# regeirk/pycwt

Hardware: NVIDIA H100
Metric: cwt_scale_points_per_sec (higher is better)
Workload: dtype f64

## Files before the change

### pycwt_b200/csrc/cplx.cuh

```cuda
#pragma once
#include <cuda_runtime.h>

#ifndef HD
#ifdef CWTB_HOST_EMU
#define HD inline
#else
#define HD __host__ __device__ __forceinline__
#endif
#endif

namespace cwtb {

template <typename T> struct Vec2;
template <> struct Vec2<double> { using type = double2; };
template <> struct Vec2<float> { using type = float2; };
template <typename T> using cx = typename Vec2<T>::type;

template <typename T> HD cx<T> mk(T a, T b) {
  cx<T> r; r.x = a; r.y = b; return r;
}
template <typename V> HD V cadd(V a, V b) { a.x += b.x; a.y += b.y; return a; }
template <typename V> HD V csub(V a, V b) { a.x -= b.x; a.y -= b.y; return a; }
template <typename V> HD V cmul(V a, V b) {
  V r;
  r.x = a.x * b.x - a.y * b.y;
  r.y = a.x * b.y + a.y * b.x;
  return r;
}
template <typename V> HD V cconj(V a) { a.y = -a.y; return a; }
template <int SIGN, typename V> HD V mul_si(V a) {
  V r;
  if (SIGN > 0) { r.x = -a.y; r.y = a.x; } else { r.x = a.y; r.y = -a.x; }
  return r;
}
template <typename V, typename T> HD V cscale(V a, T s) { a.x *= s; a.y *= s; return a; }

HD void sincospi_hd(double x, double *s, double *c) {
#if defined(__CUDA_ARCH__) && !defined(CWTB_HOST_EMU)
  sincospi(x, s, c);
#else
  ::sincos(3.14159265358979323846 * x, s, c);
#endif
}

HD void sincos_hd(double x, double *s, double *c) {
#if defined(__CUDA_ARCH__) && !defined(CWTB_HOST_EMU)
  sincos(x, s, c);
#else
  ::sincos(x, s, c);
#endif
}

HD double norm2_rn(double re, double im) {
#if defined(__CUDA_ARCH__) && !defined(CWTB_HOST_EMU)
  return __dadd_rn(__dmul_rn(re, re), __dmul_rn(im, im));
#else
  return re * re + im * im;
#endif
}

template <int SIGN, typename V> HD void dft2(V &a, V &b) {
  V t = csub(a, b);
  a = cadd(a, b);
  b = t;
}

template <int SIGN, typename V>
HD void dft4(V &x0, V &x1, V &x2, V &x3) {
  V t0 = cadd(x0, x2), t1 = csub(x0, x2);
  V t2 = cadd(x1, x3), t3 = mul_si<SIGN>(csub(x1, x3));
  x0 = cadd(t0, t2);
  x2 = csub(t0, t2);
  x1 = cadd(t1, t3);
  x3 = csub(t1, t3);
}

template <int SIGN, typename T, typename V> HD V mul_w8_1(V a) {
  const T h = (T)0.70710678118654752440;
  V r;
  if (SIGN > 0) { r.x = (a.x - a.y) * h; r.y = (a.x + a.y) * h; }
  else          { r.x = (a.x + a.y) * h; r.y = (a.y - a.x) * h; }
  return r;
}
template <int SIGN, typename T, typename V> HD V mul_w8_3(V a) {
  const T h = (T)0.70710678118654752440;
  V r;
  if (SIGN > 0) { r.x = (-a.x - a.y) * h; r.y = (a.x - a.y) * h; }
  else          { r.x = (a.y - a.x) * h; r.y = (-a.x - a.y) * h; }
  return r;
}
// ... 76 lines not shown
```

### pycwt_b200/csrc/engine.cu

```cuda
#include <algorithm>
#include <array>
#include <cmath>
#include <cstdint>
#include <cstdio>
#include <cstdlib>
#include <cstring>
#include <map>
#include <mutex>
#include <set>
#include <string>
#include <type_traits>
#include <vector>

#include <cuda_runtime.h>
#include <dlfcn.h>
#include <initializer_list>

#include "../../include/cwt_b200.h"
#include "kernels.cuh"

using namespace cwtb;

template <class B, class = void> struct BodyNT { static constexpr int value = NT; };
template <class B> struct BodyNT<B, std::void_t<decltype(B::NTB)>> { static constexpr int value = B::NTB; };
// ... 1435 lines not shown
                 &c->C, &c->A12, &c->F, &c->aux, &c->rowd, &c->win, &c->mask, &c->hist, &c->noise, &c->wide, &c->blueA, &c->blueX, &c->blueY, &c->pspec, &c->prot, &c->coh.buf, &c->cross.buf, &c->coh3.buf, &c->coh.counts, &c->coh3.counts})
    if (b->p) rt_free(b->p);
  for (auto &kv : c->ntabs) { rt_free(kv.second.hi); rt_free(kv.second.lo); }
  for (auto &kv : c->blue) { rt_free(kv.second.wm); rt_free(kv.second.bf[0]); rt_free(kv.second.bf[1]); }
  if (c->tw64) rt_free(c->tw64);
  if (c->tw32) rt_free(c->tw32);
  for (void *p : c->pinned) rt_host_free(p);
  for (void *p : c->devallocs) rt_free(p);
  rt_event_destroy(c->e0);
  rt_event_destroy(c->e1);
  rt_stream_destroy(c->stream);
  for (auto &st : c->copy_streams) rt_stream_destroy(st);
  rt_stream_destroy(c->aux_stream);
  rt_stream_destroy(c->prio_stream);
  rt_stream_destroy(c->prio_short);
  rt_event_destroy(c->ev_angle);
  rt_event_destroy(c->ev_coarse);
  rt_event_destroy(c->ev_coarse_short);
  for (auto &ev : c->ev_h2d) rt_event_destroy(ev);
  for (auto &ev : c->ev_used) rt_event_destroy(ev);
  for (void *p : c->stage_host) if (p) rt_host_free(p);
  for (auto &st : c->chain_streams) rt_stream_destroy(st);
  for (auto &ev : c->ev_joinc) rt_event_destroy(ev);
  rt_event_destroy(c->ev_fork);
  rt_event_destroy(c->ev_join);
  delete c;
}

const char *cwtb_last_error(cwtb_ctx *c) { return c ? c->err.c_str() : "null context"; }

int cwtb_set_band_eps(cwtb_ctx *c, double eps) {
  if (!c || !(eps >= 0) || eps >= 1e-6) return fail(c, CWTB_ERR_ARG, "band eps must be in [0, 1e-6)");
  c->band_eps = eps;
  return 0;
}

int cwtb_set_expand_eps(cwtb_ctx *c, double eps64, double eps32) {
  if (!c || !(eps64 >= 0) || !(eps32 >= 0) || eps64 > 1e-6 || eps32 > 1e-3)
    return fail(c, CWTB_ERR_ARG, "expansion tolerance must be in [0, 1e-6] (fp64) / [0, 1e-3] (fp32)");
  c->expand_eps = eps64;
  c->expand_eps32 = eps32;
  return 0;
}

int cwtb_host_alloc(cwtb_ctx *c, size_t bytes, void **out) {
  if (!c || !out) return CWTB_ERR_ARG;
  if (rt_host_alloc(out, bytes) != 0) return fail(c, CWTB_ERR_NOMEM, "pinned allocation failed");
  c->pinned.insert(*out);
  return 0;
}
int cwtb_host_free(cwtb_ctx *c, void *p) {
  if (!c || !c->pinned.count(p)) return CWTB_ERR_ARG;
  c->pinned.erase(p);
  rt_host_free(p);
  return 0;
}
int cwtb_dev_alloc(cwtb_ctx *c, size_t bytes, void **out) {
  if (!c || !out) return CWTB_ERR_ARG;
  if (rt_malloc(out, bytes) != 0) return fail(c, CWTB_ERR_NOMEM, "device allocation failed");
  c->devallocs.insert(*out);
  return 0;
}
int cwtb_dev_free(cwtb_ctx *c, void *p) {
  if (!c || !c->devallocs.count(p)) return CWTB_ERR_ARG;
  c->devallocs.erase(p);
  rt_free(p);
  return 0;
}
int cwtb_memcpy_h2d(cwtb_ctx *c, void *dst, const void *src, size_t bytes) {
  RT(rt_h2d(dst, src, bytes, c->stream));
  RT(rt_sync(c->stream));
  return 0;
}
int cwtb_memcpy_d2h(cwtb_ctx *c, void *dst, const void *src, size_t bytes) {
  RT(rt_d2h(dst, src, bytes, c->stream));
  RT(rt_sync(c->stream));
  return 0;
}
int cwtb_sync(cwtb_ctx *c) {
  RT(rt_sync(c->stream));
  return 0;
}

static const double kOsUs = 9.5;
static const double kTwoKernelUs = 23.2;

struct DevTmp {
  void *p = nullptr;
  ~DevTmp() { if (p) rt_free(p); }
};

static int os_plan(cwtb_ctx *c, const Job &job, double dt, int family, double param, std::vector<OsRow> &os) {
  constexpr int L = OsBody<4>::L, GR = 4;
  auto os_cheaper = [](int M) { return M <= L / 2 && kOsUs * L / (double)(L - M + 1) < kTwoKernelUs; };
  os.assign(job.S, OsRow());
  const unsigned N = job.N;
  if (!c->os_on || job.precision != CWTB_F64 || job.exact || family == CWTB_TABLE ||
      !(c->band_eps > 0) || !(c->expand_eps > 0) || N < 2u * L)
    return 0;
  const long long half = (long long)N / 2;
  std::vector<int> cand;
  std::vector<double> cs;
  for (const ScaleDesc &d : job.descs) {
    if (d.chan != 0 || d.k_hi < d.k_lo || d.k_lo <= -half || d.k_hi >= ((long long)N - 1) / 2) continue;
    if (d.ip_log2Nc || (d.log2K <= 10 || (d.log2K <= DIRECT_MAX_LOG2 && d.log2K < job.log2N))) continue;
    cand.push_back(d.row);
    cs.push_back(d.s);
  }
  if (cand.empty()) return 0;
  const int nc = (int)cand.size();
  const size_t wcap = (size_t)job.S * job.nbatch * job.n0;
  const int chunk = (int)std::max<size_t>(1, wcap / N);
  int e = ensure(c, c->W, std::max<size_t>((size_t)chunk * N, wcap) * sizeof(double2));
  if (e) return e;
  double2 *h = (double2 *)c->W.p;
  DevTmp dimp, part;
  if (rt_malloc(&dimp.p, (size_t)N * sizeof(double))) return fail(c, CWTB_ERR_NOMEM, "device allocation failed");
  {
    std::vector<double> delta(N, 0.0);
    delta[0] = 1.0;
    RT(rt_h2d(dimp.p, delta.data(), (size_t)N * sizeof(double), c->stream));
    RT(rt_sync(c->stream));
  }
  const int nblk = 64;
  if (rt_malloc(&part.p, (size_t)chunk * nblk * sizeof(double))) return fail(c, CWTB_ERR_NOMEM, "device allocation failed");
  std::vector<double> farmax(nc, 0.0);
  std::vector<double2> win((size_t)nc * 2 * L);
  for (int r0 = 0; r0 < nc; r0 += chunk) {
    const int nr = std::min(chunk, nc - r0);
    Job imp;
    const double xeps = c->expand_eps;
    c->expand_eps = 0;
    e = build_job(c, imp, (long long)N, dt, cs.data() + r0, nr, family, param, CWTB_F64, false, 1);
    c->expand_eps = xeps;
    if (e) return e;
    if ((e = upload_descs(c, imp))) return e;
    if ((e = run_job<double>(c, imp, (const double *)dimp.p, h, EPI_STORE))) return e;
    if (N > 2u * L) {
      AbsMaxArgs aa{h, (double *)part.p, (long long)N, (long long)L, (long long)N - L, nblk};
      if ((e = launch<AbsMaxBody>(c, nblk, nr, aa))) return e;
      std::vector<double> ph((size_t)nr * nblk);
      RT(rt_d2h(ph.data(), part.p, ph.size() * sizeof(double), c->stream));
      RT(rt_sync(c->stream));
      for (int r = 0; r < nr; ++r)
        for (int b = 0; b < nblk; ++b) farmax[r0 + r] = std::max(farmax[r0 + r], ph[(size_t)r * nblk + b]);
    }
    for (int r = 0; r < nr; ++r) {
      RT(rt_d2h(&win[(size_t)(r0 + r) * 2 * L], h + (size_t)r * N + (N - L), L * sizeof(double2), c->stream));
      RT(rt_d2h(&win[(size_t)(r0 + r) * 2 * L + L], h + (size_t)r * N, L * sizeof(double2), c->stream));
    }
    RT(rt_sync(c->stream));
  }
  struct Acc { int r, t0, t1; };
  std::vector<Acc> acc;
  std::vector<double> m(2 * L), pre(2 * L + 1);
  for (int r = 0; r < nc; ++r) {
    const double2 *w = &win[(size_t)r * 2 * L];
    double mx = farmax[r];
    for (int i = 0; i < 2 * L; ++i) mx = std::max(mx, std::max(std::fabs(w[i].x), std::fabs(w[i].y)));
    const double ulp = 2.220446049250313e-16 * mx;
    if (!(mx > 0) || farmax[r] > 128 * ulp) continue;
    const double floor_ = std::max(2 * farmax[r], 8 * ulp);
    double l1 = 0;
    pre[0] = 0;
    for (int i = 0; i < 2 * L; ++i) {
      const double a = std::hypot(w[i].x, w[i].y);
      l1 += a;
      m[i] = std::max(std::fabs(w[i].x), std::fabs(w[i].y)) > floor_ ? a : 0.0;
// ... 1846 lines not shown
```

### pycwt_b200/csrc/fft_tile.cuh

```cuda
#pragma once
#include "cplx.cuh"

namespace cwtb {

#ifndef CWTB_NT
#define CWTB_NT 128
#endif
#ifndef CWTB_NT_F32
#define CWTB_NT_F32 256
#endif
#ifndef CWTB_TILE_F64
#define CWTB_TILE_F64 4096
#endif
#ifndef CWTB_TILE_F32
#define CWTB_TILE_F32 8192
#endif
#ifndef CWTB_MINB
#define CWTB_MINB 1
#endif
#ifndef CWTB_UNROLL_B
#define CWTB_UNROLL_B 1
#endif
#define CWTB_STR_(x) #x
#define CWTB_STR(x) CWTB_STR_(x)
// ... 265 lines not shown
  }
  HD void load(int, V (&x)[R]) {
    if (ONE_SHOT) {
      V e = nroot_t<T>(nt, (unsigned)base * pp);
      const V se = nroot_t<T>(nt, (unsigned)stride * pp);
      const V ne = nroot_t<T>(nt, (unsigned)(-K) * pp);
#pragma unroll
      for (int i = 0; i < R; ++i) {
        const int r = base + i * stride;
        x[i] = cmul(ldg(&B[r]), (r >= rsplit) ? cmul(e, ne) : e);
        e = cmul(e, se);
      }
      return;
    }
#pragma unroll
    for (int i = 0; i < R; ++i) { x[i] = a[ONE_SHOT ? 0 : i]; a[ONE_SHOT ? 0 : i] = cmul(a[ONE_SHOT ? 0 : i], d[ONE_SHOT ? 0 : i]); }
  }
};

template <typename T, int K, int L, int R, int SIGN, class Loader, bool ROWS = false>
HD void pass_mid(cx<T> *sm, const cx<T> *__restrict__ tw, Loader &ld, int tid) {
  using V = cx<T>;
  using LY = Lay<T, K, ROWS>;
  constexpr int NT = TileCfg<T>::NT;
  constexpr int Ln = L / R, I = K / R, P = LY::P;
  constexpr int LANES = (I >= NT) ? NT : I;
  constexpr int GROUPS = NT / LANES;
  const int tp0 = tid % LANES, bg = tid / LANES;
  for (int tp = tp0; tp < I; tp += LANES) {
    const int g = tp / Ln, j = tp % Ln;
    V twv[R];
#pragma unroll
    static_assert(tw_radix(L) == R, "pass twiddle table was built for another radix");
    for (int c = 1; c < R; ++c) {
      V w = ldg(&tw[tw_offset(L) + (c - 1) * Ln + j]);
      if (SIGN < 0) w.y = -w.y;
      twv[c] = w;
    }
    ld.begin(g * L + j, Ln, bg, GROUPS);
    CWTB_PRAGMA_UNROLL_B
    for (int b = bg; b < P; b += GROUPS) {
      V x[R];
      ld.load(b, x);
      dftR<R, SIGN, T>(x);
#pragma unroll
      for (int c = 1; c < R; ++c) x[c] = cmul(x[c], twv[c]);
#pragma unroll
      for (int c = 0; c < R; ++c) sm[LY::phys(b, g * L + c * Ln + j)] = x[c];
    }
  }
}

template <typename T, int K, int SIGN, class Storer, bool ROWS = false, bool GMAJOR = false>
HD void pass_last(const cx<T> *sm, Storer &st, int tid) {
  using V = cx<T>;
  using LY = Lay<T, K, ROWS>;
  constexpr int NT = TileCfg<T>::NT;
  constexpr int R = Plan<K>::RL, G = K / R, P = LY::P;
  for (int idx = tid; idx < G * P; idx += NT) {
    const int b = GMAJOR ? idx / G : idx % P, g = GMAJOR ? idx % G : idx / P;
    V x[R];
#pragma unroll
    for (int i = 0; i < R; ++i) x[i] = sm[LY::phys(b, g * R + i)];
    dftR<R, SIGN, T>(x);
    st.store(b, Plan<K>::qlow(g), G, x);
  }
}

template <typename T, int K> struct TilePhases {
  static constexpr int NP = Plan<K>::NP;
};

template <typename T, int K, int SIGN, class Loader, bool ROWS = false>
HD void tile_first(cx<T> *sm, const cx<T> *tw, Loader &ld, int tid) {
  pass_mid<T, K, K, Plan<K>::R1, SIGN, Loader, ROWS>(sm, tw, ld, tid);
}
template <typename T, int K, int SIGN, bool ROWS = false>
HD void tile_second(cx<T> *sm, const cx<T> *tw, int tid) {
  SmemLoader<T, K, ROWS> ld;
  ld.sm = sm;
  pass_mid<T, K, K / Plan<K>::R1, Plan<K>::R2, SIGN, SmemLoader<T, K, ROWS>, ROWS>(sm, tw, ld, tid);
}

}
```

### pycwt_b200/csrc/kernels.cuh

```cuda
#pragma once
#include <math.h>
#include "fft_tile.cuh"

namespace cwtb {

struct ScaleDesc {
  double s;
  double amp;
  int row;
  int k_lo, k_hi;
  int log2K;
  int rsplit;
  int trow;
  int chan;
  int pad_;
  long long boff;
  int ip_log2Nc;
  int ip_kc;
  int ip_w;
  int os_grp;
  long long ip_coff;
  long long ip_woff;
  double ip_beta;
  double ip_dc;
// ... 252 lines not shown
            for (int r1 = 0; r1 < K1; ++r1)
              acc = cadd(acc, cmul(bv[r1], wt[(b * 2 + (neg[r1] ? 1 : 0)) * K1 + r1]));
            sm[LY::phys(b, r2)] = cmul(acc, t);
            t = cmul(t, dr);
          }
          e = cmul(e, se);
          dr = cmul(dr, sdr);
        }
      } else
      for (int it0 = 0; it0 < NIT; it0 += IB) {
        V bv[IB][K1], t[IB], dd[IB];
#pragma unroll
        for (int q = 0; q < IB; ++q) {
          const int r2 = tid + NT * (it0 + q);
#pragma unroll
          for (int r1 = 0; r1 < K1; ++r1) bv[q][r1] = ldg(&B[r1 * K + r2]);
          t[q] = e;
          dd[q] = dr;
          e = cmul(e, se);
          dr = cmul(dr, sdr);
        }
#pragma unroll
        for (int b = 0; b < P; ++b) {
          V acc[IB];
#pragma unroll
          for (int q = 0; q < IB; ++q) acc[q] = mk<T>(0, 0);
#pragma unroll
          for (int r1 = 0; r1 < K1; ++r1) {
            if (r1 != r1s) {
              const V w = wt[(b * 2 + (r1 > r1s ? 1 : 0)) * K1 + r1];
#pragma unroll
              for (int q = 0; q < IB; ++q) acc[q] = cadd(acc[q], cmul(bv[q][r1], w));
            } else {
              const V wp = wt[(b * 2 + 0) * K1 + r1], wn = wt[(b * 2 + 1) * K1 + r1];
#pragma unroll
              for (int q = 0; q < IB; ++q) {
                const bool neg = (tid + NT * (it0 + q)) >= r2s;
                acc[q] = cadd(acc[q], cmul(bv[q][r1], neg ? wn : wp));
              }
            }
          }
#pragma unroll
          for (int q = 0; q < IB; ++q) {
            sm[LY::phys(b, tid + NT * (it0 + q))] = cmul(acc[q], t[q]);
            t[q] = cmul(t[q], dd[q]);
          }
        }
      }
    } else if constexpr (PH == 2) {
      SmemLoader<T, K> ld;
      ld.sm = sm;
      tile_first<T, K, +1>(sm, a.tw, ld, tid);
    } else if constexpr (PH == 3 && NP == 3) {
      tile_second<T, K, +1>(sm, a.tw, tid);
    } else {
      OutStorer<T> st;
      st.row = a.W + (size_t)d.row * a.n0;
      st.nout = a.n0;
      st.u0 = u0;
      st.U = U;
      st.epi.mode = a.epi;
      pass_last<T, K, +1>(sm, st, tid);
    }
  }
};

template <typename T> struct PassBArgs {
  const cx<T> *Z;
  cx<T> *out;
  const cx<T> *tw;
  const ScaleDesc *descs;
  const double *grow;
  long long pitch, nout;
  double post;
  unsigned N;
  int first, row0;
  int epi;
  int pf_dist;
  int ny;
  int by0;
  int ileave;
};

template <typename T, int SIGN, int K2 = K2C> struct PassBBody {
  static constexpr int NTB = TileCfg<T>::NT;
  static constexpr int NT = NTB;
  using V = cx<T>;
  using Args = PassBArgs<T>;
  static constexpr int K = K2;
  using LY = Lay<T, K, true>;
  static constexpr int NP = Plan<K>::NP;
  static constexpr int NPHASE = NP + 1;
  static constexpr size_t SMEM = LY::TILE_BYTES + 16;
  static constexpr bool ROWS_ALIGNED = (LY::PITCH * sizeof(V)) % 16 == 0;
  template <int PH> HD static void phase(const Args &a, int bx, int by, int tid, void *smraw) {
    static_assert(ROWS_ALIGNED, "PassB: tile rows must start on 16-byte boundaries");
    const int ey = by;
    by = a.ny - 1 - ey;
    V *sm = (V *)smraw;
    const int U = (int)(a.N / K);
    const int u0 = bx * LY::P;
    TileBarrier tb;
    tb.bar = (unsigned long long *)((char *)smraw + LY::TILE_BYTES);
    if constexpr (PH == 0) {
      const int nvalid = (U - u0) < LY::P ? (U - u0) : LY::P;
      const V *src = a.Z + (size_t)by * a.N + (size_t)u0 * K;
      if (tid == 0) {
        tb.init_and_expect((unsigned)(nvalid * K * sizeof(V)));
        for (int b = 0; b < nvalid; ++b)
          tb.copy(sm + LY::phys(b, 0), src + (size_t)b * K, (unsigned)(K * sizeof(V)));
      }
      if (tid == 0 && a.pf_dist > 0) {
        long long t = (long long)bx + a.pf_dist;
        int pe = ey;
        const int tiles = (U + LY::P - 1) / LY::P;
        while (t >= tiles && pe + 1 < a.ny) { t -= tiles; ++pe; }
        const int py = a.ny - 1 - pe;
        if (t < tiles && t * LY::P + LY::P <= U)
          TileBarrier::prefetch_l2(a.Z + (size_t)py * a.N + (size_t)t * LY::P * K,
                                   (unsigned)(LY::P * K * sizeof(V)));
      }
      for (int b = nvalid; b < LY::P; ++b)
        for (int i = tid; i < K; i += NT) sm[LY::phys(b, i)] = mk<T>(0, 0);
    } else if constexpr (PH == 1) {
      tb.wait(0);
      SmemLoader<T, K, true> ld;
      ld.sm = sm;
      tile_first<T, K, SIGN, SmemLoader<T, K, true>, true>(sm, a.tw, ld, tid);
    } else if constexpr (PH == 2 && NP == 3) {
      tile_second<T, K, SIGN, true>(sm, a.tw, tid);
    } else {
      const int il = a.ileave > 1 ? a.ileave : 1;
      const int outer = (a.by0 + by) / il;
      const int row = a.descs ? a.descs[a.first + outer].row : a.row0 + outer;
      OutStorer<T> st;
      st.row = a.out + (size_t)row * a.pitch;
      st.nout = a.nout;
      st.u0 = u0;
      st.U = U;
      st.ostride = il;
      st.ooff = (a.by0 + by) % il;
      st.epi.mode = a.epi;
      if (a.epi == EPI_GAUSS) {
        st.epi.g = a.grow[row];
        st.epi.invn = 1.0 / ((double)a.N * il);
        st.epi.post = a.post;
        st.epi.nfreq = (long long)a.N * il;
      }
      pass_last<T, K, SIGN, OutStorer<T>, true>(sm, st, tid);
      if (tid == 0) tb.inval();
    }
  }
};

struct OsGroup {
  int first, count;
  int t1, hop;
  long long hoff;
};
struct OsArgs {
  const ScaleDesc *descs;
  const OsGroup *groups;
  const double *sig;
  const double2 *H;
  double2 *W;
  const double2 *tw;
  long long n0;
  unsigned N;
  int epi;
};

template <int L, int R> struct OsSigLoader {
  const double *x;
  long long start, n0;
  unsigned nmask;
  int hop, base, stride;
  HD void begin(int base_, int stride_, int, int) { base = base_; stride = stride_; }
  HD void load(int b, double2 (&v)[R]) const {
    const long long s = start + (long long)b * hop + base;
#pragma unroll
    for (int i = 0; i < R; ++i) {
      const long long n = (s + (long long)i * stride) & (long long)nmask;
      v[i] = make_double2(n < n0 ? ldg(&x[n]) : 0.0, 0.0);
    }
  }
};
template <int L> struct OsHalfStorer {
  double2 *xs;
  template <int R> HD void store(int b, int ql, int qs, double2 (&x)[R]) const {
#pragma unroll
    for (int c = 0; c < R; ++c) {
      const int q = ql + c * qs;
      if (q <= L / 2) xs[b * (L / 2 + 1) + q] = x[c];
    }
  }
};
template <int L, int R> struct OsSpecLoader {
  const double2 *xs, *H;
  int base, stride;
  double2 hv[R];
  HD void begin(int base_, int stride_, int, int) {
    base = base_; stride = stride_;
#pragma unroll
    for (int i = 0; i < R; ++i) hv[i] = ldg(&H[base + i * stride]);
  }
  HD void load(int b, double2 (&v)[R]) const {
#pragma unroll
    for (int i = 0; i < R; ++i) {
      const int q = base + i * stride;
      const double2 y = q <= L / 2 ? xs[b * (L / 2 + 1) + q] : cconj(xs[b * (L / 2 + 1) + L - q]);
      v[i] = cmul(y, hv[i]);
    }
  }
};
struct OsStorer {
  double2 *row;
  long long nb0, n0;
  int t1, hop, epi;
  template <int R> HD void store(int b, int ql, int qs, double2 (&x)[R]) const {
    const long long nb = nb0 + (long long)b * hop;
#pragma unroll
    for (int c = 0; c < R; ++c) {
      const int i = ql + c * qs;
      const long long n = nb + i;
      if (i >= t1 && i < t1 + hop && n < n0) {
        if (epi == EPI_STORE) st_stream(&row[n], x[c]);
        else row[n] = cmul(row[n], cconj(x[c]));
      }
    }
  }
};

template <int G> struct OsBody {
  static constexpr int L = 1024;
  static constexpr int NTB = TileCfg<double>::NT;
  static constexpr int NT = NTB;
  using Args = OsArgs;
  using LY = Lay<double, L>;
  static constexpr int P = LY::P;
  static_assert(Plan<L>::NP == 3, "overlap-save phases assume a three-pass tile plan");
  static constexpr int NPHASE = 3 + 3 * G;
  static constexpr size_t SMEM = LY::TILE_BYTES + (size_t)P * (L / 2 + 1) * sizeof(double2);
  template <int PH> HD static void phase(const Args &a, int bx, int by, int tid, void *smraw) {
    double2 *sm = (double2 *)smraw;
    double2 *xs = (double2 *)((char *)smraw + LY::TILE_BYTES);
    const OsGroup g = a.groups[by];
    const long long n_first = (long long)bx * P * g.hop;
    if (n_first >= a.n0) return;
    if constexpr (PH == 0) {
      OsSigLoader<L, Plan<L>::R1> ld;
      ld.x = a.sig + (size_t)a.descs[g.first].chan * a.n0; ld.start = n_first - g.t1; ld.n0 = a.n0; ld.nmask = a.N - 1; ld.hop = g.hop;
      tile_first<double, L, -1>(sm, a.tw, ld, tid);
    } else if constexpr (PH == 1) {
      tile_second<double, L, -1>(sm, a.tw, tid);
    } else if constexpr (PH == 2) {
      OsHalfStorer<L> st{xs};
      pass_last<double, L, -1, OsHalfStorer<L>, false, true>(sm, st, tid);
    } else {
      constexpr int r = (PH - 3) / 3, step = (PH - 3) % 3;
      if (r >= g.count) return;
      if constexpr (step == 0) {
        OsSpecLoader<L, Plan<L>::R1> ld;
        ld.xs = xs; ld.H = a.H + g.hoff + (long long)r * L;
        tile_first<double, L, +1>(sm, a.tw, ld, tid);
      } else if constexpr (step == 1) {
        tile_second<double, L, +1>(sm, a.tw, tid);
      } else {
        OsStorer st;
        st.row = a.W + (size_t)a.descs[g.first + r].row * a.n0;
        st.nb0 = n_first - g.t1; st.n0 = a.n0; st.t1 = g.t1; st.hop = g.hop; st.epi = a.epi;
        pass_last<double, L, +1, OsStorer, false, true>(sm, st, tid);
      }
    }
  }
};

struct AbsMaxArgs { const double2 *h; double *out; long long pitch, lo, hi; int nblk; };
struct AbsMaxBody {
  using Args = AbsMaxArgs;
  static constexpr int NPHASE = 2;
  static constexpr size_t SMEM = NT * sizeof(double);
  template <int PH> HD static void phase(const Args &a, int bx, int by, int tid, void *smraw) {
    double *sm = (double *)smraw;
    if constexpr (PH == 0) {
      const long long chunk = (a.hi - a.lo + a.nblk - 1) / a.nblk;
      const long long s = a.lo + bx * chunk, e = s + chunk < a.hi ? s + chunk : a.hi;
      double m = 0;
      for (long long i = s + tid; i < e; i += NT) {
        const double2 v = a.h[(size_t)by * a.pitch + i];
        m = fmax(m, fmax(fabs(v.x), fabs(v.y)));
      }
      sm[tid] = m;
    } else if (tid == 0) {
      double m = 0;
      for (int i = 0; i < NT; ++i) m = fmax(m, sm[i]);
      a.out[(size_t)by * a.nblk + bx] = m;
    }
  }
};

enum { MODE_DENSE = 0, MODE_BAND = 1, MODE_REAL = 2, MODE_CPLX = 3, MODE_COARSE = 4 };

template <typename T> HD cx<T> coarse_value(const Fam &fam, const ScaleDesc &d, const cx<T> *spec, int r, unsigned Nx) {
  const int Nc = 1 << d.ip_log2Nc;
  const int kp = r < Nc / 2 ? r : r - Nc;
  const int k = d.ip_kc + kp;
  if (k < d.k_lo || k > d.k_hi) return mk<T>(0, 0);
  const cx<T> b = band_value<T>(fam, d, spec, (unsigned)k & (Nx - 1), k, Nx);
  const double pw = 3.14159265358979323846 * (double)d.ip_w;
  const double x = pw * ((double)kp / (double)Nc);
  const double bb = d.ip_beta * d.ip_beta;
  const double z = sqrt(fma(-x, x, bb));
  const double f = d.ip_dc * (z / sinh(z));
  return mk<T>((T)((double)b.x * f), (T)((double)b.y * f));
}

template <typename T> struct PassAArgs {
  const ScaleDesc *descs;
  const cx<T> *spec;
  const cx<T> *Bbuf;
  const void *in;
  cx<T> *Z;
  const cx<T> *tw;
  Fam fam;
  NTab nt;
  long long in_pitch, n_in;
  unsigned N;
  int first, row0;
  int pf_dist;
  unsigned K2;
  unsigned Nx;
};

template <typename T, int K1, int MODE, int SIGN> struct PassABody {
  static constexpr int NTB = TileCfg<T>::NT;
  static constexpr int NT = NTB;
  using V = cx<T>;
  using Args = PassAArgs<T>;
  using LY = Lay<T, K1>;
  static constexpr int NP = Plan<K1>::NP;
  static constexpr int P = LY::P;
  static constexpr int T2 = P < K2C ? P : K2C;
  static constexpr int NPHASE = NP == 1 ? 1 : NP + 1;
  static constexpr size_t SMEM = LY::BYTES;

  struct Src {
    const Args &a;
    ScaleDesc d;
    int by, p;
    V twist0;
    HD Src(const Args &a_, int by_, int p_) : a(a_), by(by_), p(p_) {
      if (MODE == MODE_DENSE || MODE == MODE_BAND || MODE == MODE_COARSE) d = a.descs[a.first + by];
    }
    HD V get(int pos, int r2) const {
      const unsigned r = (unsigned)pos * a.K2 + (unsigned)r2;
      if (MODE == MODE_DENSE) {
        const int k = (int)r - (r >= a.N / 2 ? (int)a.N : 0);
        if (a.fam.family != 3 && (k < d.k_lo || k > d.k_hi)) return mk<T>(0, 0);
        return band_value<T>(a.fam, d, a.spec, r, k, a.N);
      } else if (MODE == MODE_BAND) {
        V v = ldg(&a.Bbuf[d.boff + r]);
        if (p == 0 || NP > 1) return v;
        const int k1 = pos - ((int)r >= d.rsplit ? K1 : 0);
        V w = nroot_t<T>(a.nt, (unsigned)k1 * (unsigned)p * a.K2);
        return cmul(v, w);
      } else if (MODE == MODE_COARSE) {
        return coarse_value<T>(a.fam, d, a.spec, (int)r, a.Nx);
      } else if (MODE == MODE_REAL) {
        const T *row = (const T *)a.in + (size_t)(a.row0 + by) * a.in_pitch;
        return mk<T>((long long)r < a.n_in ? ldg(&row[r]) : (T)0, (T)0);
      } else {
        const V *row = (const V *)a.in + (size_t)(a.row0 + by) * a.in_pitch;
        return (long long)r < a.n_in ? ldg(&row[r]) : mk<T>(0, 0);
      }
    }
  };

  template <int PH> HD static void phase(const Args &a, int bx, int by, int tid, void *smraw) {
    V *sm = (V *)smraw;
    const int NTILE2 = (int)(a.K2 / T2);
    const int p = bx / NTILE2;
    const int r20 = (bx % NTILE2) * T2;
    const int M = (int)(a.N / ((unsigned)K1 * a.K2));
    ZStorer<T, SIGN> st;
    st.Z = a.Z + (size_t)by * a.N;
    st.nt = a.nt;
    st.p = p;
    st.M = M;
    st.r20 = r20;
    st.bmax = T2;
    st.K2 = a.K2;
    if constexpr (NP == 1) {
      Src src(a, by, p);
      for (int b = tid; b < T2; b += NT) {
        V x[K1];
#pragma unroll
        for (int i = 0; i < K1; ++i) x[i] = src.get(i, r20 + b);
        dftR<K1, SIGN, T>(x);
        st.store(b, 0, 1, x);
      }
    } else if constexpr (PH == 0) {
      Src src(a, by, p);
      if (MODE == MODE_BAND && a.pf_dist > 0 && T2 * sizeof(V) >= 256) {
        const int tiles = M * NTILE2;
        const int t = bx + a.pf_dist;
        if (t < tiles) {
          const int r20n = (t % NTILE2) * T2;
          const V *base = a.Bbuf + src.d.boff + r20n;
          for (int pos = tid; pos < K1; pos += NT)
            TileBarrier::prefetch_l2(base + (size_t)pos * a.K2, (unsigned)(T2 * sizeof(V)));
        }
      }
      if (MODE == MODE_CPLX && a.pf_dist > 0 && T2 * sizeof(V) >= 256) {
        const int t = bx + a.pf_dist;
        if (t < M * NTILE2) {
          const V *row = (const V *)a.in + (size_t)(a.row0 + by) * a.in_pitch + (t % NTILE2) * T2;
          for (int pos = tid; pos < K1; pos += NT)
            if ((long long)pos * a.K2 + (t % NTILE2) * T2 + T2 <= a.n_in)
              TileBarrier::prefetch_l2(row + (size_t)pos * a.K2, (unsigned)(T2 * sizeof(V)));
        }
      }
      if (MODE == MODE_DENSE && a.fam.family == 0 && T2 <= NT) {
        constexpr int DPOS = NT / T2;
        const ScaleDesc &d = src.d;
        const int b = tid % T2;
        const long long D = (long long)DPOS * a.K2;
        const double wd = 6.283185307179586 * ((double)D * a.fam.dw);
        const double aa = d.s * wd;
        const double q = exp(-aa * aa);
        double g = 0, rho = 0;
        long long kprev = 0;
        int since = 1 << 30;
        constexpr int UB = CWTB_PASSA_BATCH;
        const V *sp = a.spec + (size_t)d.chan * a.N + (unsigned)(r20 + b);
        for (int pos0 = tid / T2; pos0 < K1; pos0 += DPOS * UB) {
          V raw[UB];
          int kk[UB];
#pragma unroll
          for (int u = 0; u < UB; ++u) {
            const int pos = pos0 + u * DPOS;
            const unsigned r = (unsigned)pos * a.K2 + (unsigned)(r20 + b);
            const int k = (int)r - (r >= a.N / 2 ? (int)a.N : 0);
            const bool in = pos < K1 && k >= d.k_lo && k <= d.k_hi;
            kk[u] = in ? k : (int)0x7fffffff;
            raw[u] = in ? ldg(&sp[(size_t)pos * a.K2]) : mk<T>(0, 0);
          }
#pragma unroll
          for (int u = 0; u < UB; ++u) {
            const int pos = pos0 + u * DPOS;
            if (pos >= K1) break;
            V v = mk<T>(0, 0);
            if (kk[u] != (int)0x7fffffff) {
              const int k = kk[u];
              if (since >= 16 || (long long)k != kprev + D || g < 1e-290) {
                const double f = d.s * (6.283185307179586 * ((double)k * a.fam.dw));
                const double dd = f - a.fam.f0;
                g = exp(-0.5 * dd * dd);
                rho = exp(-aa * dd - 0.5 * aa * aa);
                since = 0;
              } else {
                g *= rho;
                rho *= q;
                ++since;
              }
              kprev = k;
              v = cscale(raw[u], (T)(g * d.amp));
            } else {
              since = 1 << 30;
            }
            sm[LY::phys(b, pos)] = v;
          }
        }
      } else {
        CWTB_PRAGMA_UNROLL_A
        for (int idx = tid; idx < K1 * T2; idx += NT) {
          const int b = idx % T2, pos = idx / T2;
          sm[LY::phys(b, pos)] = src.get(pos, r20 + b);
        }
      }
    } else if constexpr (PH == 1) {
      if (MODE == MODE_BAND && p != 0) {
        SmemTwistLoader<T, K1, Plan<K1>::R1> ld;
        ld.sm = sm;
        ld.nt = a.nt;
        ld.rsplit_row = a.descs[a.first + by].rsplit / (int)a.K2;
        ld.pk2 = (unsigned)p * a.K2;
        tile_first<T, K1, SIGN>(sm, a.tw, ld, tid);
      } else {
        SmemLoader<T, K1> ld;
        ld.sm = sm;
        tile_first<T, K1, SIGN>(sm, a.tw, ld, tid);
      }
    } else if constexpr (PH == 2 && NP == 3) {
      tile_second<T, K1, SIGN>(sm, a.tw, tid);
    } else {
      pass_last<T, K1, SIGN>(sm, st, tid);
    }
  }
};

struct CoarseSeg { int first, count, log2Nc, cta0; };
constexpr int CSEG_MAX = 32;
HD constexpr size_t cmax(size_t a, size_t b) { return a > b ? a : b; }
template <typename T> struct CoarseArgs {
  const ScaleDesc *descs;
  const cx<T> *spec;
  cx<T> *Z;
  cx<T> *C;
  const cx<T> *tw;
  Fam fam;
  NTab nt[11];
  unsigned Nx;
  int nseg;
  int pf_dist;
  CoarseSeg seg[CSEG_MAX];
};
template <typename T> HD const CoarseSeg &coarse_seg(const CoarseArgs<T> &a, int bx) {
  int s = 0;
  while (s + 1 < a.nseg && bx >= a.seg[s + 1].cta0) ++s;
  return a.seg[s];
}

template <typename T> struct CoarseRowsBody {
  static constexpr int NTB = TileCfg<T>::NT;
  static constexpr int NT = NTB;
  using V = cx<T>;
  using Args = CoarseArgs<T>;
  template <int K> static constexpr size_t bytes() { return Lay<T, K>::BYTES; }
  static constexpr size_t SMEM = cmax(cmax(cmax(bytes<64>(), bytes<128>()), cmax(bytes<256>(), bytes<512>())), bytes<1024>());
  static constexpr int NPHASE = 4;
  HD static int ctas(int log2Nc, int rows) {
    const int P = TileCfg<T>::TILE >> log2Nc;
    return (rows + P - 1) / P;
  }
  struct Storer {
    V *out;
    int nb;
    int K;
    template <int R> HD void store(int b, int ql, int qs, V (&x)[R]) const {
      if (b >= nb) return;
#pragma unroll
      for (int c = 0; c < R; ++c) out[(size_t)b * K + ql + c * qs] = x[c];
    }
  };
  template <int K, int PH> HD static void tile(const Args &a, const CoarseSeg &g, int bx, int tid, V *sm) {
    using LY = Lay<T, K>;
    constexpr int NP = Plan<K>::NP;
    static_assert(NP >= 2, "coarse rows: multi-pass tile plans only");
    const int row0 = (bx - g.cta0) * LY::P;
    const int nb = g.count - row0 < LY::P ? g.count - row0 : LY::P;
    if constexpr (PH == 0) {
      for (int idx = tid; idx < LY::P * K; idx += NT) {
        const int b = idx / K, pos = idx % K;
        V v = mk<T>(0, 0);
        if (b < nb) v = coarse_value<T>(a.fam, a.descs[g.first + row0 + b], a.spec, pos, a.Nx);
        sm[LY::phys(b, pos)] = v;
      }
    } else if constexpr (PH == 1) {
      SmemLoader<T, K> ld;
      ld.sm = sm;
      tile_first<T, K, +1>(sm, a.tw, ld, tid);
    } else if constexpr (PH == 2 && NP == 3) {
      tile_second<T, K, +1>(sm, a.tw, tid);
    } else if constexpr (PH == NP) {
      Storer st{a.C + a.descs[g.first].ip_coff + (size_t)row0 * K, nb, K};
      pass_last<T, K, +1>(sm, st, tid);
    }
  }
  template <int PH> HD static void phase(const Args &a, int bx, int, int tid, void *smraw) {
    const CoarseSeg &g = coarse_seg(a, bx);
    V *sm = (V *)smraw;
    switch (g.log2Nc) {
      case 6: tile<64, PH>(a, g, bx, tid, sm); break;
      case 7: tile<128, PH>(a, g, bx, tid, sm); break;
      case 8: tile<256, PH>(a, g, bx, tid, sm); break;
      case 9: tile<512, PH>(a, g, bx, tid, sm); break;
      case 10: tile<1024, PH>(a, g, bx, tid, sm); break;
    }
  }
};

template <typename T> struct CoarseABody {
  static constexpr int NTB = TileCfg<T>::NT;
  static constexpr int NT = NTB;
  using V = cx<T>;
  using Args = CoarseArgs<T>;
  template <int K1> using A = PassABody<T, K1, MODE_COARSE, +1>;
  static constexpr size_t SMEM = cmax(cmax(cmax(cmax(A<2>::SMEM, A<4>::SMEM), cmax(A<8>::SMEM, A<16>::SMEM)),
                                           cmax(cmax(A<32>::SMEM, A<64>::SMEM), cmax(A<128>::SMEM, A<256>::SMEM))),
                                      cmax(A<512>::SMEM, A<1024>::SMEM));
  static constexpr int NPHASE = 4;
  template <int K1> HD static int per_row() { return K2C / A<K1>::T2; }
  HD static int ctas(int log2Nc, int rows) {
    switch (log2Nc - 10) {
      case 1: return rows * per_row<2>();
      case 2: return rows * per_row<4>();
      case 3: return rows * per_row<8>();
      case 4: return rows * per_row<16>();
      case 5: return rows * per_row<32>();
      case 6: return rows * per_row<64>();
      case 7: return rows * per_row<128>();
      case 8: return rows * per_row<256>();
      case 9: return rows * per_row<512>();
      case 10: return rows * per_row<1024>();
    }
    return 0;
  }
  template <int K1, int PH> HD static void tile(const Args &a, const CoarseSeg &g, int bx, int tid, void *sm) {
    if constexpr (PH < A<K1>::NPHASE) {
      const int local = bx - g.cta0, per = per_row<K1>();
      PassAArgs<T> pa{};
      pa.descs = a.descs; pa.spec = a.spec; pa.tw = a.tw; pa.fam = a.fam; pa.nt = a.nt[g.log2Nc - 10];
      pa.Z = a.Z + a.descs[g.first].ip_coff;
      pa.N = 1u << g.log2Nc; pa.Nx = a.Nx; pa.first = g.first; pa.K2 = K2C;
      A<K1>::template phase<PH>(pa, local % per, local / per, tid, sm);
    }
  }
  template <int PH> HD static void phase(const Args &a, int bx, int, int tid, void *sm) {
    const CoarseSeg &g = coarse_seg(a, bx);
    switch (g.log2Nc - 10) {
      case 1: tile<2, PH>(a, g, bx, tid, sm); break;
      case 2: tile<4, PH>(a, g, bx, tid, sm); break;
      case 3: tile<8, PH>(a, g, bx, tid, sm); break;
      case 4: tile<16, PH>(a, g, bx, tid, sm); break;
      case 5: tile<32, PH>(a, g, bx, tid, sm); break;
      case 6: tile<64, PH>(a, g, bx, tid, sm); break;
      case 7: tile<128, PH>(a, g, bx, tid, sm); break;
      case 8: tile<256, PH>(a, g, bx, tid, sm); break;
      case 9: tile<512, PH>(a, g, bx, tid, sm); break;
      case 10: tile<1024, PH>(a, g, bx, tid, sm); break;
    }
  }
};

template <typename T> struct CoarseBBody {
  using B = PassBBody<T, +1>;
  static constexpr int NTB = B::NTB;
  static constexpr int NT = NTB;
  using Args = CoarseArgs<T>;
  static constexpr size_t SMEM = B::SMEM;
  static constexpr int NPHASE = B::NPHASE;
  HD static int per_row(int log2Nc) {
    constexpr int P = B::LY::P;
    return ((1 << (log2Nc - 10)) + P - 1) / P;
  }
  HD static int ctas(int log2Nc, int rows) { return rows * per_row(log2Nc); }
  template <int PH> HD static void phase(const Args &a, int bx, int, int tid, void *sm) {
    const CoarseSeg &g = coarse_seg(a, bx);
    const int local = bx - g.cta0, per = per_row(g.log2Nc);
    const long long off = a.descs[g.first].ip_coff;
    const unsigned Nc = 1u << g.log2Nc;
    PassBArgs<T> pb{};
    pb.Z = a.Z + off; pb.out = a.C + off; pb.tw = a.tw;
    pb.pitch = Nc; pb.nout = Nc; pb.N = Nc; pb.post = 1.0;
    pb.epi = EPI_STORE; pb.pf_dist = a.pf_dist; pb.ny = g.count; pb.ileave = 1;
    B::template phase<PH>(pb, local % per, local / per, tid, sm);
  }
};

template <typename T> struct ExpandArgs {
  const ScaleDesc *descs;
  const cx<T> *C;
  const double *wt;
  cx<T> *W;
  NTab nt;
  long long n0;
  unsigned N;
  int first;
  int epi;
  int log2N;
};

template <typename T, int TAPS, int EPI = EPI_STORE> struct ExpandBody {
  static constexpr int NTB = TileCfg<T>::NT;
  static constexpr int NT = NTB;
  static constexpr int MINB = sizeof(T) == 8 ? 4 : 2;
  using V = cx<T>;
  using Args = ExpandArgs<T>;
  static constexpr int L = 32;
  static constexpr int MINR = 4;
  static constexpr int MAXRUN = NT / MINR;
  static constexpr int STAGE = MAXRUN * L + TAPS;
  HD static int skew(int i) { return i + (i >> 5); }
  static constexpr int NPHASE = 2;
  static constexpr size_t SMEM = (size_t)(STAGE + STAGE / 32 + 2) * sizeof(V);
  template <int PH> HD static void phase(const Args &a, int bx, int by, int tid, void *smraw) {
    V *sm = (V *)smraw;
    const ScaleDesc &d = a.descs[a.first + by];
    const int log2R = a.log2N - d.ip_log2Nc;
    const int R = 1 << log2R;
    const int Nc = 1 << d.ip_log2Nc;
    const int RB = R < NT ? R : NT;
    const int NRUN = NT / RB;
    const int MT = NRUN * L;
    const int mtiles = (Nc + MT - 1) / MT;
    const int mt = bx % mtiles, rb = bx / mtiles;
    if (rb * RB >= R) return;
    const int m0 = mt * MT;
    if constexpr (PH == 0) {
      const V *c = a.C + d.ip_coff;
      for (int i = tid; i < MT + TAPS; i += NT) {
        const int m = (m0 - (TAPS / 2 - 1) + i) & (Nc - 1);
        sm[skew(i)] = ldg(&c[m]);
      }
    } else {
      const int rl = tid & (RB - 1), j = tid / RB;
      const int rho = rb * RB + rl;
      const int ms = m0 + j * L;
      const long long nfirst = ((long long)ms << log2R) + rho;
      long long keep = (a.n0 - nfirst + R - 1) >> log2R;
      if (keep > Nc - ms) keep = Nc - ms;
      const int smax = keep < 0 ? 0 : (keep > L ? L : (int)keep);
      if (smax == 0) return;
      T hw[TAPS];
      const double *wt = a.wt + d.ip_woff + rho;
#pragma unroll
      for (int t = 0; t < TAPS; ++t) hw[t] = (T)ldg(&wt[(size_t)t * R]);
      const V *run = sm + 33 * j;
      V win[TAPS];
// ... 1423 lines not shown
```

Baseline: 110.2 billion.

## Use register-resident 32x32 FFT core for 1024-point fp64 tiles

Adds a register-resident 1024-point FFT core (radix-32 in registers, one shared-memory transpose with padded rows and fused twiddles) and uses it in the dense pass A, pass B, and the overlap-save kernel in place of the three-pass shared-memory tile plan. This cuts phases and block barriers per tile and shrinks shared-memory traffic. In exchange each thread holds 32 complex doubles, which raises register pressure, and some helpers are marked noinline to keep code size down. The overlap-save cost constants are retuned so the planner picks overlap-save more often.

```diff
diff --git a/profiles/micro/x32_ab.py b/profiles/micro/x32_ab.py
--- /dev/null
+++ b/profiles/micro/x32_ab.py
@@ -0,0 +1,81 @@
+import os
+import subprocess
+import sys
+
+import numpy as np
+
+ROOT = os.path.dirname(os.path.dirname(os.path.dirname(os.path.abspath(__file__))))
+sys.path.insert(0, ROOT)
+import workloads as wl
+from pycwt_b200 import _engine
+from bench import pin_to_gpu_numa_node
+
+CORE = (("OsBody", "OsBody<4>"), ("dense first", "PassABody<double, 1024, 0, 1>"),
+        ("second", "PassBBody<double, 1, 1024"))
+
+
+def main():
+    args = sys.argv[1:]
+    parent = args[0]
+    new = args[1] if len(args) > 1 and not args[1].isdigit() else os.path.join(ROOT, "pycwt_b200", "libcwtb200.so")
+    rounds = int(args[-1]) if args[-1].isdigit() else 8
+    pin_to_gpu_numa_node(0)
+    print(subprocess.run(["nvidia-smi", "--query-gpu=name,power.limit,clocks.max.sm", "--format=csv"],
+                         capture_output=True, text=True).stdout.strip())
+    c = wl.C2
+    x = wl.config2_signal()
+    sj = wl.config2_scales()
+    arms = {"parent": _engine.Engine(0, lib_path=parent), "new": _engine.Engine(0, lib_path=new)}
+    dev = {}
+    for name, eng in arms.items():
+        d = eng.dev_alloc(x.nbytes)
+        eng.h2d(d, x)
+        eng.cwt_dev(d, 0, c["n"], c["dt"], sj, _engine.MORLET, c["f0"], _engine.F64)
+        eng.bench_last(10)
+        dev[name] = d
+        plan = eng.last_plan(len(sj))
+        os_rows = [j for j, p in enumerate(plan) if p == -2]
+        print("%-6s plan: %d overlap-save rows (%s), %d expansion, %d exact" % (
+            name, len(os_rows), "%d..%d" % (os_rows[0], os_rows[-1]) if os_rows else "-",
+            sum(p < -2 for p in plan), sum(p >= 0 for p in plan)))
+    times = {k: [] for k in arms}
+    for _ in range(rounds):
+        for name, eng in arms.items():
+            times[name].append(eng.bench_last(20))
+    for name, t in times.items():
+        print("%-6s config 2 step %.4f ms (min %.4f, max %.4f) over %d runs of 20 steps" % (
+            name, float(np.median(t)), min(t), max(t), len(t)))
+    print("median difference parent - new: %.4f ms" % (float(np.median(times["parent"])) - float(np.median(times["new"]))))
+    prof = {name: eng.profile_last() for name, eng in arms.items()}
+    for label, key in CORE:
+        for name in arms:
+            ks = [k for k in prof[name] if k["name"].startswith(key)]
+            ms = sum(k["ms"] for k in ks)
+            rows = sum(k["rows"] for k in ks)
+            print("%-11s %-6s %7.4f ms serialised, %3d rows, %5.1f us per row" % (
+                label, name, ms, rows, 1e3 * ms / rows if rows else float("nan")))
+    for name in arms:
+        print(name + ": serialised kernels of one step")
+        for k in sorted(prof[name], key=lambda k: -k["ms"]):
+            print("      %-52s %3d x  %7.4f ms  rows %d" % (k["name"], k["launches"], k["ms"], k["rows"]))
+    err = []
+    for r0 in range(0, len(sj), 32):
+        rows = []
+        for eng in arms.values():
+            out = np.empty((32, c["n"]), np.complex128)
+            eng._check(eng.lib.cwtb_get_w(eng.h, _engine._ptr(out), 1, r0, 32))
+            rows.append(out)
+        for i in range(32):
+            err.append(float(np.abs(rows[1][i] - rows[0][i]).max() / np.abs(rows[0][i]).max()))
+    err = np.array(err)
+    print("per row max|W_new - W_parent| / max|W_parent| of the row: worst %.2e (row %d); rows 0..63 worst %.2e, "
+          "rows 64.. worst %.2e, rows bit-identical %d of %d" % (
+              err.max(), int(err.argmax()), err[:64].max(), err[64:].max(), int((err == 0).sum()), len(err)))
+    print("per row, rows 0..63: " + " ".join("%.1e" % e for e in err[:64]))
+    for name, eng in arms.items():
+        eng.dev_free(dev[name])
+        eng.close()
+
+
+if __name__ == "__main__":
+    main()
diff --git a/pycwt_b200/csrc/cplx.cuh b/pycwt_b200/csrc/cplx.cuh
--- a/pycwt_b200/csrc/cplx.cuh
+++ b/pycwt_b200/csrc/cplx.cuh
@@ -4,8 +4,10 @@
 #ifndef HD
 #ifdef CWTB_HOST_EMU
 #define HD inline
+#define HD_NOINLINE inline
 #else
 #define HD __host__ __device__ __forceinline__
+#define HD_NOINLINE __host__ __device__ __noinline__
 #endif
 #endif
 
diff --git a/pycwt_b200/csrc/engine.cu b/pycwt_b200/csrc/engine.cu
--- a/pycwt_b200/csrc/engine.cu
+++ b/pycwt_b200/csrc/engine.cu
@@ -1541,8 +1541,8 @@
   return 0;
 }
 
-static const double kOsUs = 9.5;
-static const double kTwoKernelUs = 23.2;
+static const double kOsUs = 7.0;
+static const double kTwoKernelUs = 23.5;
 
 struct DevTmp {
   void *p = nullptr;
diff --git a/pycwt_b200/csrc/fft_tile.cuh b/pycwt_b200/csrc/fft_tile.cuh
--- a/pycwt_b200/csrc/fft_tile.cuh
+++ b/pycwt_b200/csrc/fft_tile.cuh
@@ -371,4 +371,73 @@
   pass_mid<T, K, K / Plan<K>::R1, Plan<K>::R2, SIGN, SmemLoader<T, K, ROWS>, ROWS>(sm, tw, ld, tid);
 }
 
-}
+enum { X32_BMAJOR = 0, X32_WARP = 1 };
+struct X32 {
+  static constexpr int K = 1024, C = 32, P = 4;
+  static_assert(TileCfg<double>::NT == P * C && TileCfg<double>::TILE == P * K,
+                "the register-resident core assumes a 4096-element fp64 tile in 128 threads");
+  template <int MAP> HD static void map(int tid, int &b, int &col) {
+    if (MAP == X32_BMAJOR) { b = tid % P; col = tid / P; } else { b = tid / C; col = tid % C; }
+  }
+};
+struct X32Ex {
+  static constexpr int ROW = 33, BP = 32 * ROW + 2;
+  static constexpr size_t BYTES = (size_t)X32::P * BP * sizeof(double2);
+  HD static int at(int b, int n1, int k1) { return b * BP + n1 * ROW + k1; }
+};
+template <bool ROWS> struct X32InTile {
+  HD static int at(int b, int n1, int k1) { return Lay<double, X32::K, ROWS>::phys(b, n1 + 32 * k1); }
+};
+
+template <int SIGN, class EX>
+HD void x32_exchange_out(double2 *ex, const double2 *__restrict__ tw, int b, int n1, double2 (&x)[32]) {
+  dftR<32, SIGN, double>(x);
+  double2 wa[4];
+#pragma unroll
+  for (int a = 1; a < 4; ++a) {
+    wa[a] = ldg(&tw[tw_offset(256) + (a - 1) * 64 + 2 * n1]);
+    if (SIGN < 0) wa[a].y = -wa[a].y;
+  }
+#pragma unroll
+  for (int c = 0; c < 8; ++c) {
+    double2 wc = mk<double>(1.0, 0.0);
+    if (c > 0) {
+      wc = ldg(&tw[tw_offset(1024) + (c - 1) * 128 + n1]);
+      if (SIGN < 0) wc.y = -wc.y;
+    }
+#pragma unroll
+    for (int a = 0; a < 4; ++a) {
+      const int k1 = 8 * a + c;
+      if (k1 > 0) {
+        const double2 w = a == 0 ? wc : (c == 0 ? wa[a] : cmul(wc, wa[a]));
+        x[k1] = cmul(x[k1], w);
+      }
+      ex[EX::at(b, n1, k1)] = x[k1];
+    }
+  }
+}
+template <int SIGN, int MAP, class EX, class Loader>
+HD void x32_first(double2 *ex, const double2 *tw, Loader &ld, int tid) {
+  int b, n1;
+  X32::map<MAP>(tid, b, n1);
+  double2 x[32];
+  ld.begin(n1, 32, b, X32::P);
+  ld.load(b, x);
+  x32_exchange_out<SIGN, EX>(ex, tw, b, n1, x);
+}
+template <int SIGN, int MAP, class EX, class Storer>
+HD void x32_last(const double2 *ex, Storer &st, int tid) {
+  int b, k1;
+  X32::map<MAP>(tid, b, k1);
+  double2 y[32];
+#pragma unroll
+  for (int n1 = 0; n1 < 32; ++n1) y[n1] = ex[EX::at(b, n1, k1)];
+  dftR<32, SIGN, double>(y);
+  double2 lo[16], hi[16];
+#pragma unroll
+  for (int c = 0; c < 16; ++c) { lo[c] = y[c]; hi[c] = y[c + 16]; }
+  st.store(b, k1, 32, lo);
+  st.store(b, k1 + 512, 32, hi);
+}
+
+}
diff --git a/pycwt_b200/csrc/kernels.cuh b/pycwt_b200/csrc/kernels.cuh
--- a/pycwt_b200/csrc/kernels.cuh
+++ b/pycwt_b200/csrc/kernels.cuh
@@ -358,7 +358,7 @@
   int ileave;
 };
 
-template <typename T, int SIGN, int K2 = K2C> struct PassBBody {
+template <typename T, int SIGN, int K2 = K2C, bool REG = (sizeof(T) == 8 && K2 == X32::K)> struct PassBBody {
   static constexpr int NTB = TileCfg<T>::NT;
   static constexpr int NT = NTB;
   using V = cx<T>;
@@ -366,7 +366,7 @@
   static constexpr int K = K2;
   using LY = Lay<T, K, true>;
   static constexpr int NP = Plan<K>::NP;
-  static constexpr int NPHASE = NP + 1;
+  static constexpr int NPHASE = REG ? 3 : NP + 1;
   static constexpr size_t SMEM = LY::TILE_BYTES + 16;
   static constexpr bool ROWS_ALIGNED = (LY::PITCH * sizeof(V)) % 16 == 0;
   template <int PH> HD static void phase(const Args &a, int bx, int by, int tid, void *smraw) {
@@ -402,8 +402,11 @@
       tb.wait(0);
       SmemLoader<T, K, true> ld;
       ld.sm = sm;
-      tile_first<T, K, SIGN, SmemLoader<T, K, true>, true>(sm, a.tw, ld, tid);
-    } else if constexpr (PH == 2 && NP == 3) {
+      if constexpr (REG)
+        x32_first<SIGN, X32_WARP, X32InTile<true>>(sm, a.tw, ld, tid);
+      else
+        tile_first<T, K, SIGN, SmemLoader<T, K, true>, true>(sm, a.tw, ld, tid);
+    } else if constexpr (PH == 2 && NP == 3 && !REG) {
       tile_second<T, K, SIGN, true>(sm, a.tw, tid);
     } else {
       const int il = a.ileave > 1 ? a.ileave : 1;
@@ -423,7 +426,10 @@
         st.epi.post = a.post;
         st.epi.nfreq = (long long)a.N * il;
       }
-      pass_last<T, K, SIGN, OutStorer<T>, true>(sm, st, tid);
+      if constexpr (REG)
+        x32_last<SIGN, X32_BMAJOR, X32InTile<true>>(sm, st, tid);
+      else
+        pass_last<T, K, SIGN, OutStorer<T>, true>(sm, st, tid);
       if (tid == 0) tb.inval();
     }
   }
@@ -508,46 +514,45 @@
 };
 
 template <int G> struct OsBody {
-  static constexpr int L = 1024;
+  static constexpr int L = X32::K;
   static constexpr int NTB = TileCfg<double>::NT;
   static constexpr int NT = NTB;
   using Args = OsArgs;
-  using LY = Lay<double, L>;
-  static constexpr int P = LY::P;
-  static_assert(Plan<L>::NP == 3, "overlap-save phases assume a three-pass tile plan");
-  static constexpr int NPHASE = 3 + 3 * G;
-  static constexpr size_t SMEM = LY::TILE_BYTES + (size_t)P * (L / 2 + 1) * sizeof(double2);
+  static constexpr int P = X32::P;
+  static constexpr int NPHASE = 2 + 2 * G;
+  static constexpr size_t SMEM = X32Ex::BYTES + (size_t)P * (L / 2 + 1) * sizeof(double2);
   template <int PH> HD static void phase(const Args &a, int bx, int by, int tid, void *smraw) {
-    double2 *sm = (double2 *)smraw;
-    double2 *xs = (double2 *)((char *)smraw + LY::TILE_BYTES);
+    double2 *ex = (double2 *)smraw;
+    double2 *xs = (double2 *)((char *)smraw + X32Ex::BYTES);
     const OsGroup g = a.groups[by];
     const long long n_first = (long long)bx * P * g.hop;
     if (n_first >= a.n0) return;
     if constexpr (PH == 0) {
-      OsSigLoader<L, Plan<L>::R1> ld;
+      OsSigLoader<L, X32::C> ld;
       ld.x = a.sig + (size_t)a.descs[g.first].chan * a.n0; ld.start = n_first - g.t1; ld.n0 = a.n0; ld.nmask = a.N - 1; ld.hop = g.hop;
-      tile_first<double, L, -1>(sm, a.tw, ld, tid);
+      x32_first<-1, X32_WARP, X32Ex>(ex, a.tw, ld, tid);
     } else if constexpr (PH == 1) {
-      tile_second<double, L, -1>(sm, a.tw, tid);
-    } else if constexpr (PH == 2) {
       OsHalfStorer<L> st{xs};
-      pass_last<double, L, -1, OsHalfStorer<L>, false, true>(sm, st, tid);
+      x32_last<-1, X32_WARP, X32Ex>(ex, st, tid);
     } else {
-      constexpr int r = (PH - 3) / 3, step = (PH - 3) % 3;
+      constexpr int r = (PH - 2) / 2;
       if (r >= g.count) return;
-      if constexpr (step == 0) {
-        OsSpecLoader<L, Plan<L>::R1> ld;
-        ld.xs = xs; ld.H = a.H + g.hoff + (long long)r * L;
-        tile_first<double, L, +1>(sm, a.tw, ld, tid);
-      } else if constexpr (step == 1) {
-        tile_second<double, L, +1>(sm, a.tw, tid);
-      } else {
-        OsStorer st;
-        st.row = a.W + (size_t)a.descs[g.first + r].row * a.n0;
-        st.nb0 = n_first - g.t1; st.n0 = a.n0; st.t1 = g.t1; st.hop = g.hop; st.epi = a.epi;
-        pass_last<double, L, +1, OsStorer, false, true>(sm, st, tid);
-      }
-    }
+      if constexpr (PH % 2 == 0) inv_first(a, g, r, n_first, ex, xs, tid);
+      else inv_last(a, g, r, n_first, ex, tid);
+    }
+  }
+  HD_NOINLINE static void inv_first(const Args &a, const OsGroup &g, int r, long long n_first, double2 *ex,
+                                    const double2 *xs, int tid) {
+    OsSpecLoader<L, X32::C> ld;
+    ld.xs = xs; ld.H = a.H + g.hoff + (long long)r * L;
+    x32_first<+1, X32_WARP, X32Ex>(ex, a.tw, ld, tid);
+  }
+  HD_NOINLINE static void inv_last(const Args &a, const OsGroup &g, int r, long long n_first, const double2 *ex,
+                                   int tid) {
+    OsStorer st;
+    st.row = a.W + (size_t)a.descs[g.first + r].row * a.n0;
+    st.nb0 = n_first - g.t1; st.n0 = a.n0; st.t1 = g.t1; st.hop = g.hop; st.epi = a.epi;
+    x32_last<+1, X32_WARP, X32Ex>(ex, st, tid);
   }
 };
 
@@ -617,8 +622,61 @@
   static constexpr int NP = Plan<K1>::NP;
   static constexpr int P = LY::P;
   static constexpr int T2 = P < K2C ? P : K2C;
-  static constexpr int NPHASE = NP == 1 ? 1 : NP + 1;
-  static constexpr size_t SMEM = LY::BYTES;
+  static constexpr bool REG = sizeof(T) == 8 && K1 == X32::K && MODE == MODE_DENSE;
+  static constexpr int NPHASE = REG ? 2 : (NP == 1 ? 1 : NP + 1);
+  static constexpr size_t SMEM = REG ? X32Ex::BYTES : LY::BYTES;
+
+  static constexpr int DPOS = NT / T2 > 0 ? NT / T2 : 1;
+  static constexpr int UB = CWTB_PASSA_BATCH;
+  struct GaussWalk {
+    const Args &a;
+    const ScaleDesc &d;
+    unsigned rb;
+    const V *sp;
+    long long D;
+    double aa, q, g = 0, rho = 0;
+    long long kprev = 0;
+    int since = 1 << 30;
+    HD GaussWalk(const Args &a_, const ScaleDesc &d_, int r20, int b) : a(a_), d(d_), rb((unsigned)(r20 + b)) {
+      sp = a.spec + (size_t)d.chan * a.N + rb;
+      D = (long long)DPOS * a.K2;
+      const double wd = 6.283185307179586 * ((double)D * a.fam.dw);
+      aa = d.s * wd;
+      q = exp(-aa * aa);
+    }
+    HD void load(int pos0, V (&raw)[UB], int (&kk)[UB]) const {
+#pragma unroll
+      for (int u = 0; u < UB; ++u) {
+        const int pos = pos0 + u * DPOS;
+        const unsigned r = (unsigned)pos * a.K2 + rb;
+        const int k = (int)r - (r >= a.N / 2 ? (int)a.N : 0);
+        const bool in = pos < K1 && k >= d.k_lo && k <= d.k_hi;
+        kk[u] = in ? k : (int)0x7fffffff;
+        raw[u] = in ? ldg(&sp[(size_t)pos * a.K2]) : mk<T>(0, 0);
+      }
+    }
+    HD_NOINLINE static double2 seed(double s, double dw, double f0, double aa, int k) {
+      const double f = s * (6.283185307179586 * ((double)k * dw));
+      const double dd = f - f0;
+      return make_double2(exp(-0.5 * dd * dd), exp(-aa * dd - 0.5 * aa * aa));
+    }
+    HD V next(V raw, int kk) {
+      if (kk == (int)0x7fffffff) { since = 1 << 30; return mk<T>(0, 0); }
+      const int k = kk;
+      if (since >= 16 || (long long)k != kprev + D || g < 1e-290) {
+        const double2 gr = seed(d.s, a.fam.dw, a.fam.f0, aa, k);
+        g = gr.x;
+        rho = gr.y;
+        since = 0;
+      } else {
+        g *= rho;
+        rho *= q;
+        ++since;
+      }
+      kprev = k;
+      return cscale(raw, (T)(g * d.amp));
+    }
+  };
 
   struct Src {
     const Args &a;
@@ -652,6 +710,8 @@
     }
   };
 
+  HD_NOINLINE static V get_out_of_line(const Args &a, int by, int p, int pos, int r2) { return Src(a, by, p).get(pos, r2); }
+
   template <int PH> HD static void phase(const Args &a, int bx, int by, int tid, void *smraw) {
     V *sm = (V *)smraw;
     const int NTILE2 = (int)(a.K2 / T2);
@@ -675,6 +735,30 @@
         dftR<K1, SIGN, T>(x);
         st.store(b, 0, 1, x);
       }
+    } else if constexpr (REG) {
+      if constexpr (PH == 0) {
+        static_assert(T2 == X32::P && DPOS == X32::C && X32::K % (DPOS * UB) == 0, "dense fill vs core columns");
+        Src src(a, by, p);
+        const int b = tid % T2, n1 = tid / T2;
+        V x[X32::C];
+        if (a.fam.family == 0) {
+          GaussWalk gw(a, src.d, r20, b);
+#pragma unroll
+          for (int it = 0; it < X32::C / UB; ++it) {
+            V raw[UB];
+            int kk[UB];
+            gw.load(n1 + it * UB * DPOS, raw, kk);
+#pragma unroll
+            for (int u = 0; u < UB; ++u) x[it * UB + u] = gw.next(raw[u], kk[u]);
+          }
+        } else {
+#pragma unroll
+          for (int i = 0; i < X32::C; ++i) x[i] = get_out_of_line(a, by, p, n1 + DPOS * i, r20 + b);
+        }
+        x32_exchange_out<SIGN, X32Ex>(sm, a.tw, b, n1, x);
+      } else {
+        x32_last<SIGN, X32_BMAJOR, X32Ex>(sm, st, tid);
+      }
     } else if constexpr (PH == 0) {
       Src src(a, by, p);
       if (MODE == MODE_BAND && a.pf_dist > 0 && T2 * sizeof(V) >= 256) {
@@ -697,54 +781,17 @@
         }
       }
       if (MODE == MODE_DENSE && a.fam.family == 0 && T2 <= NT) {
-        constexpr int DPOS = NT / T2;
-        const ScaleDesc &d = src.d;
         const int b = tid % T2;
-        const long long D = (long long)DPOS * a.K2;
-        const double wd = 6.283185307179586 * ((double)D * a.fam.dw);
-        const double aa = d.s * wd;
-        const double q = exp(-aa * aa);
-        double g = 0, rho = 0;
-        long long kprev = 0;
-        int since = 1 << 30;
-        constexpr int UB = CWTB_PASSA_BATCH;
-        const V *sp = a.spec + (size_t)d.chan * a.N + (unsigned)(r20 + b);
+        GaussWalk gw(a, src.d, r20, b);
         for (int pos0 = tid / T2; pos0 < K1; pos0 += DPOS * UB) {
           V raw[UB];
           int kk[UB];
-#pragma unroll
-          for (int u = 0; u < UB; ++u) {
-            const int pos = pos0 + u * DPOS;
-            const unsigned r = (unsigned)pos * a.K2 + (unsigned)(r20 + b);
-            const int k = (int)r - (r >= a.N / 2 ? (int)a.N : 0);
-            const bool in = pos < K1 && k >= d.k_lo && k <= d.k_hi;
-            kk[u] = in ? k : (int)0x7fffffff;
-            raw[u] = in ? ldg(&sp[(size_t)pos * a.K2]) : mk<T>(0, 0);
-          }
+          gw.load(pos0, raw, kk);
 #pragma unroll
           for (int u = 0; u < UB; ++u) {
             const int pos = pos0 + u * DPOS;
             if (pos >= K1) break;
-            V v = mk<T>(0, 0);
-            if (kk[u] != (int)0x7fffffff) {
-              const int k = kk[u];
-              if (since >= 16 || (long long)k != kprev + D || g < 1e-290) {
-                const double f = d.s * (6.283185307179586 * ((double)k * a.fam.dw));
-                const double dd = f - a.fam.f0;
-                g = exp(-0.5 * dd * dd);
-                rho = exp(-aa * dd - 0.5 * aa * aa);
-                since = 0;
-              } else {
-                g *= rho;
-                rho *= q;
-                ++since;
-              }
-              kprev = k;
-              v = cscale(raw[u], (T)(g * d.amp));
-            } else {
-              since = 1 << 30;
-            }
-            sm[LY::phys(b, pos)] = v;
+            sm[LY::phys(b, pos)] = gw.next(raw[u], kk[u]);
           }
         }
       } else {
@@ -910,7 +957,7 @@
 };
 
 template <typename T> struct CoarseBBody {
-  using B = PassBBody<T, +1>;
+  using B = PassBBody<T, +1, K2C, false>;
   static constexpr int NTB = B::NTB;
   static constexpr int NT = NTB;
   using Args = CoarseArgs<T>;
```

Result: faster. 113.8 billion, median of 6 (+3.3%).
